# papuSpartan/stable-diffusion-webui-distributed

Hardware: NVIDIA H100
Metric: images/sec SD1.5 512x512 txt2img (higher is better)
Workload: dtype fp16

## Files before the change

### stable-diffusion-webui-distributed_b200/b200sd/csrc/attention_tc.cu

```cuda
#include <cstddef>
#include <cstdlib>

#include "tc_common.cuh"
#include "wgmma.cuh"
#include "b200sd_internal.h"
#include "pdl.cuh"

namespace b200sd {

constexpr int kAttnMathThreads = 256;
constexpr int kAttnThreads = kAttnMathThreads + 128;
constexpr int kQTile = 128;
constexpr int kMaxStages = 3;
constexpr uint32_t kQChunkBytes = kQTile * 128;
__host__ __device__ constexpr int kv_tile(int chunks) { return chunks == 1 ? 128 : 64; }

struct AttnParams {
  int B, heads, Sq, Skv, d, d_pad;
  int d16;
  int chunks;
  int stages;
  float scale_log2;
  void* O;
  long long ldo;
  const int* kv_len;
};

struct __align__(8) AttnShared {
  uint64_t q_full;
  uint64_t kv_full[kMaxStages];
  uint64_t kv_empty[kMaxStages];
};

template <bool kBf16>
__device__ __forceinline__ uint32_t pack_h2(float a, float b) {
  if constexpr (kBf16) {
    __nv_bfloat162 v = __floats2bfloat162_rn(a, b);
    return *reinterpret_cast<uint32_t*>(&v);
  } else {
    __half2 v = __floats2half2_rn(a, b);
    return *reinterpret_cast<uint32_t*>(&v);
  }
}

__device__ __forceinline__ void turn_wait(int wg) {
  asm volatile("bar.sync %0, %1;" ::"r"(2 + wg), "n"(kAttnMathThreads) : "memory");
}
__device__ __forceinline__ void turn_pass(int wg) {
  asm volatile("bar.arrive %0, %1;" ::"r"(3 - wg), "n"(kAttnMathThreads) : "memory");
}

template <int kKv, bool kMask>
__device__ __forceinline__ void softmax_tile(float (&s)[kKv / 2], float (&m_run)[2], float (&l_run)[2],
                                             float (&alpha)[2], float c, int valid, int colq) {
  float mx[2] = {-INFINITY, -INFINITY};
#pragma unroll
  for (int g = 0; g < kKv / 8; ++g)
#pragma unroll
    for (int h = 0; h < 2; ++h)
#pragma unroll
      for (int e = 0; e < 2; ++e) {
        float& v = s[4 * g + 2 * h + e];
        if constexpr (kMask) v = (8 * g + colq + e < valid) ? v : -INFINITY;
        mx[h] = fmaxf(mx[h], v);
      }
  float mc[2];
#pragma unroll
  for (int h = 0; h < 2; ++h) {
    mx[h] = fmaxf(mx[h], __shfl_xor_sync(0xffffffffu, mx[h], 1));
    mx[h] = fmaxf(mx[h], __shfl_xor_sync(0xffffffffu, mx[h], 2));
    const float m_new = fmaxf(m_run[h], mx[h]);
    alpha[h] = fast_exp2((m_run[h] - m_new) * c);
    m_run[h] = m_new;
    mc[h] = m_new * c;
    l_run[h] *= alpha[h];
  }
#pragma unroll
  for (int g = 0; g < kKv / 8; ++g)
#pragma unroll
    for (int h = 0; h < 2; ++h) {
      float& p0 = s[4 * g + 2 * h];
      float& p1 = s[4 * g + 2 * h + 1];
      p0 = fast_exp2(fmaf(p0, c, -mc[h]));
      p1 = fast_exp2(fmaf(p1, c, -mc[h]));
      l_run[h] += p0 + p1;
    }
}

template <int kSteps, int kKv, bool kBf16>
__device__ __forceinline__ void qk_tile(float (&s)[kKv / 2], uint64_t dq, uint64_t dk) {
#pragma unroll
  for (int ks = 0; ks < kSteps; ++ks) {
    const uint32_t off = static_cast<uint32_t>(ks & 3) * 32u;
    Wgmma<kKv, kBf16>::ss(s, dq + ((static_cast<uint32_t>(ks >> 2) * kQChunkBytes + off) >> 4),
                          dk + ((static_cast<uint32_t>(ks >> 2) * (kKv * 128u) + off) >> 4), ks != 0 ? 1u : 0u);
  }
}

template <int kChunks, bool kBf16, bool kVarlen>
__global__ void __launch_bounds__(kAttnThreads, 1)
attention_tc_kernel(const __grid_constant__ CUtensorMap tmQ, const __grid_constant__ CUtensorMap tmK,
                    const __grid_constant__ CUtensorMap tmV, const AttnParams p) {
  constexpr int kKv = kv_tile(kChunks);
  constexpr int kDv = 64 * kChunks;
  constexpr bool kOverlap = kChunks < 3;
  constexpr uint32_t kKvChunkBytes = kKv * 128;
  constexpr uint32_t kKvBytes = kChunks * kKvChunkBytes;
  extern __shared__ uint8_t smem_raw[];
  pdl_trigger();
  uint8_t* smem = reinterpret_cast<uint8_t*>((reinterpret_cast<uintptr_t>(smem_raw) + 1023) & ~uintptr_t(1023));
  uint8_t* sQ = smem;
  uint8_t* sK = sQ + kChunks * kQChunkBytes;
  uint8_t* sV = sK + p.stages * kKvBytes;
  AttnShared* sh = reinterpret_cast<AttnShared*>(sV + p.stages * kKvBytes);

  const int warp = threadIdx.x >> 5;
  const int lane = threadIdx.x & 31;
  const int qt = blockIdx.x;
  const int head = blockIdx.y;
  const int b = blockIdx.z;
  const int col0 = head * p.d_pad;

  if (threadIdx.x == kAttnMathThreads) {
    tma_prefetch_desc(&tmQ);
    tma_prefetch_desc(&tmK);
    tma_prefetch_desc(&tmV);
    mbar_init(&sh->q_full, 1);
    for (int s = 0; s < kMaxStages; ++s) {
      mbar_init(&sh->kv_full[s], 1);
      mbar_init(&sh->kv_empty[s], kAttnMathThreads / 128);
    }
    fence_mbar_init();
  }
  __syncthreads();
  pdl_wait();
  const int skv = kVarlen ? min(max(p.kv_len[b], 1), p.Skv) : p.Skv;
  const int nkv = (skv + kKv - 1) / kKv;

  if (warp >= kAttnMathThreads / 32) {
    producer_warpgroup_regs();
    if (threadIdx.x == kAttnMathThreads) {
      mbar_arrive_expect_tx(&sh->q_full, kChunks * kQChunkBytes);
#pragma unroll
      for (int c = 0; c < kChunks; ++c)
        tma_load_3d(sQ + c * kQChunkBytes, &tmQ, &sh->q_full, col0 + c * 64, qt * kQTile, b);
      for (int t = 0; t < nkv; ++t) {
        const int s = t % p.stages;
        if (t >= p.stages) mbar_wait(&sh->kv_empty[s], static_cast<uint32_t>(t / p.stages - 1) & 1u);
        mbar_arrive_expect_tx(&sh->kv_full[s], 2 * kKvBytes);
#pragma unroll
        for (int c = 0; c < kChunks; ++c) {
          tma_load_3d(sK + s * kKvBytes + c * kKvChunkBytes, &tmK, &sh->kv_full[s], col0 + c * 64, t * kKv, b);
          tma_load_3d(sV + s * kKvBytes + c * kKvChunkBytes, &tmV, &sh->kv_full[s], col0 + c * 64, t * kKv, b);
        }
      }
    }
    return;
  }

  consumer_warpgroup_regs();
  const int wg = warp >> 2;
  const int colq = (lane & 3) * 2;
  const bool signaller = (threadIdx.x & 127) == 0;
  const float c = p.scale_log2;
  const bool ragged = skv % kKv != 0;
  const uint32_t sQ_a = smem_u32(sQ) + static_cast<uint32_t>(wg) * 8192u;
  const uint32_t sK_a = smem_u32(sK), sV_a = smem_u32(sV);
  float o[kDv / 2];
#pragma unroll
  for (int i = 0; i < kDv / 2; ++i) o[i] = 0.f;
  float m_run[2] = {-INFINITY, -INFINITY}, l_run[2] = {0.f, 0.f}, alpha[2];
  float sacc[kKv / 2];
  uint32_t pa[kKv / 16][4];

  auto issue_qk = [&](int t) {
    const uint64_t dq = make_gdesc_sw128(sQ_a, 16, 1024);
    const uint64_t dk = make_gdesc_sw128(sK_a + static_cast<uint32_t>(t % p.stages) * kKvBytes, 16, 1024);
    switch (p.d16 / 16 - 4 * kChunks) {
      case -3: qk_tile<4 * kChunks - 3, kKv, kBf16>(sacc, dq, dk); break;
      case -2: qk_tile<4 * kChunks - 2, kKv, kBf16>(sacc, dq, dk); break;
      case -1: qk_tile<4 * kChunks - 1, kKv, kBf16>(sacc, dq, dk); break;
      default: qk_tile<4 * kChunks, kKv, kBf16>(sacc, dq, dk); break;
    }
    wgmma_commit();
  };
  auto issue_pv = [&](int t) {
    const uint64_t dv = make_gdesc_sw128(sV_a + static_cast<uint32_t>(t % p.stages) * kKvBytes, kKvChunkBytes, 1024);
#pragma unroll
    for (int j = 0; j < kKv / 16; ++j) Wgmma<kDv, kBf16>::rs_tb(o, pa[j], dv + static_cast<uint32_t>(j) * (2048u >> 4), 1u);
    wgmma_commit();
  };
  auto softmax = [&](int t) {
    if (ragged && t == nkv - 1) softmax_tile<kKv, true>(sacc, m_run, l_run, alpha, c, skv - t * kKv, colq);
    else softmax_tile<kKv, false>(sacc, m_run, l_run, alpha, c, 0, colq);
  };
  auto pack_p = [&]() {
#pragma unroll
    for (int g = 0; g < kKv / 8; ++g)
#pragma unroll
      for (int h = 0; h < 2; ++h) pa[g >> 1][(g & 1) * 2 + h] = pack_h2<kBf16>(sacc[4 * g + 2 * h], sacc[4 * g + 2 * h + 1]);
  };

  if (wg == 1) turn_pass(wg);
  mbar_wait(&sh->q_full, 0);
  mbar_wait(&sh->kv_full[0], 0);
  turn_wait(wg);
  wgmma_fence();
  issue_qk(0);
  turn_pass(wg);
  wgmma_wait<0>();
  reg_fence(sacc);
  softmax(0);
  pack_p();

  for (int t = 1; t < nkv; ++t) {
    mbar_wait(&sh->kv_full[t % p.stages], static_cast<uint32_t>(t / p.stages) & 1u);
    turn_wait(wg);
    reg_fence(o);
    wgmma_fence();
    if constexpr (kOverlap) {
      issue_qk(t);
      issue_pv(t - 1);
    } else {
      issue_pv(t - 1);
      wgmma_wait<0>();
      reg_fence(o);
      wgmma_fence();
      issue_qk(t);
    }
    turn_pass(wg);
    wgmma_wait<kOverlap ? 1 : 0>();
    reg_fence(sacc);
    softmax(t);
    wgmma_wait<0>();
    reg_fence(o);
    if (signaller) mbar_arrive(&sh->kv_empty[(t - 1) % p.stages]);
#pragma unroll
    for (int i = 0; i < kDv / 2; ++i) o[i] *= alpha[(i >> 1) & 1];
    pack_p();
  }

  turn_wait(wg);
  reg_fence(o);
  wgmma_fence();
  issue_pv(nkv - 1);
  if (wg == 0) turn_pass(wg);
  wgmma_wait<0>();
  reg_fence(o);
  if (signaller) mbar_arrive(&sh->kv_empty[(nkv - 1) % p.stages]);

#pragma unroll
  for (int h = 0; h < 2; ++h) {
    l_run[h] += __shfl_xor_sync(0xffffffffu, l_run[h], 1);
    l_run[h] += __shfl_xor_sync(0xffffffffu, l_run[h], 2);
  }
  const int r0 = qt * kQTile + wg * 64 + (warp & 3) * 16 + (lane >> 2);
#pragma unroll
  for (int h = 0; h < 2; ++h) {
    const int row = r0 + 8 * h;
    if (row >= p.Sq) continue;
    const float inv = 1.0f / l_run[h];
    uint8_t* orow = static_cast<uint8_t*>(p.O) + ((static_cast<long long>(b) * p.Sq + row) * p.ldo +
                                                  static_cast<long long>(head) * p.d) * 2;
#pragma unroll
    for (int g = 0; g < kDv / 8; ++g) {
      const int col = 8 * g + colq;
      if (col < p.d)
        *reinterpret_cast<uint32_t*>(orow + col * 2) = pack_h2<kBf16>(o[4 * g + 2 * h] * inv, o[4 * g + 2 * h + 1] * inv);
    }
  }
}

typedef void (*AttnKernel)(CUtensorMap, CUtensorMap, CUtensorMap, AttnParams);

template <bool kVarlen>
static AttnKernel attn_kernel_for(int chunks, int is_bf16) {
  switch (chunks * 2 + (is_bf16 ? 1 : 0)) {
    case 2: return attention_tc_kernel<1, false, kVarlen>;
    case 3: return attention_tc_kernel<1, true, kVarlen>;
    case 4: return attention_tc_kernel<2, false, kVarlen>;
    case 5: return attention_tc_kernel<2, true, kVarlen>;
    case 6: return attention_tc_kernel<3, false, kVarlen>;
    case 7: return attention_tc_kernel<3, true, kVarlen>;
    default: return nullptr;
  }
}

static int g_attn_max_smem = 0;
static bool g_attn_dev_ready[64] = {};

int attention_tc(const void* Q, long long ldq, const void* K, long long ldk, const void* V, long long ldv, void* O,
                 long long ldo, int B, int heads, int Sq, int Skv, const int* kv_len, int d, int d_pad, float scale,
                 int v_ones_col, int is_bf16, cudaStream_t stream) {
  if (B <= 0 || heads <= 0 || Sq <= 0) return B200SD_OK;
  if (Skv <= 0 || d <= 0 || d % 8 != 0 || d_pad % 16 != 0 || d_pad < d) return B200SD_ERR_INVALID;
  if (ldq % 8 || ldk % 8 || ldv % 8 || ldo % 8) return B200SD_ERR_INVALID;
  if ((reinterpret_cast<uintptr_t>(Q) | reinterpret_cast<uintptr_t>(K) | reinterpret_cast<uintptr_t>(V) |
       reinterpret_cast<uintptr_t>(O)) & 15)
    return B200SD_ERR_INVALID;
  if (ldq < static_cast<long long>(heads) * d_pad || ldk < static_cast<long long>(heads) * d_pad ||
      ldv < static_cast<long long>(heads) * d_pad || ldo < static_cast<long long>(heads) * d)
    return B200SD_ERR_INVALID;
  if (v_ones_col && d >= d_pad) return B200SD_ERR_INVALID;
  if (kv_len && (reinterpret_cast<uintptr_t>(kv_len) & 3)) return B200SD_ERR_INVALID;
  const int chunks = (((d + 15) & ~15) + 63) / 64;
  if (chunks > 3) return B200SD_ERR_UNSUPPORTED;
  {
    int dev = 0;
    if (cudaGetDevice(&dev) != cudaSuccess) return B200SD_ERR_CUDA;
    if (dev < 0 || dev >= 64) return B200SD_ERR_UNSUPPORTED;
    if (!g_attn_dev_ready[dev]) {
      int smem = 0;
      if (cudaDeviceGetAttribute(&smem, cudaDevAttrMaxSharedMemoryPerBlockOptin, dev) != cudaSuccess)
        return B200SD_ERR_CUDA;
      for (int c = 1; c <= 3; ++c)
        for (int bf = 0; bf < 2; ++bf)
          if (cudaFuncSetAttribute(attn_kernel_for<false>(c, bf), cudaFuncAttributeMaxDynamicSharedMemorySize, smem) !=
                  cudaSuccess ||
              cudaFuncSetAttribute(attn_kernel_for<true>(c, bf), cudaFuncAttributeMaxDynamicSharedMemorySize, smem) !=
                  cudaSuccess)
            return B200SD_ERR_CUDA;
      g_attn_max_smem = smem;
      g_attn_dev_ready[dev] = true;
    }
  }
  AttnParams p{};
  p.B = B; p.heads = heads; p.Sq = Sq; p.Skv = Skv; p.d = d; p.d_pad = d_pad;
  p.d16 = (d + 15) & ~15;
  p.chunks = chunks;
  p.scale_log2 = scale * 1.4426950408889634f;
  p.O = O; p.ldo = ldo;
  p.kv_len = kv_len;
  const int kv = kv_tile(chunks);
  const int nkv = (Skv + kv - 1) / kv;
  const size_t qt = static_cast<size_t>(chunks) * kQChunkBytes;
  const size_t kvt = 2 * static_cast<size_t>(chunks) * kv * 128;
  p.stages = nkv < kMaxStages ? nkv : kMaxStages;
  const size_t smem = 1024 + qt + static_cast<size_t>(p.stages) * kvt + sizeof(AttnShared);
  if (smem > static_cast<size_t>(g_attn_max_smem)) return B200SD_ERR_UNSUPPORTED;
  CUtensorMap tmQ, tmK, tmV;
  const uint32_t es[3] = {1, 1, 1};
  int rc;
  {
    const uint32_t box[3] = {64, kQTile, 1};
    const uint64_t dims[3] = {static_cast<uint64_t>(heads) * d_pad, static_cast<uint64_t>(Sq), static_cast<uint64_t>(B)};
    const uint64_t st[2] = {static_cast<uint64_t>(ldq) * 2, static_cast<uint64_t>(ldq) * 2 * Sq};
    if ((rc = make_tmap_sw128(&tmQ, Q, 3, dims, st, box, es)) != B200SD_OK) return rc;
  }
  const uint32_t kvbox[3] = {64, static_cast<uint32_t>(kv), 1};
  {
    const uint64_t dims[3] = {static_cast<uint64_t>(heads) * d_pad, static_cast<uint64_t>(Skv), static_cast<uint64_t>(B)};
    const uint64_t st[2] = {static_cast<uint64_t>(ldk) * 2, static_cast<uint64_t>(ldk) * 2 * Skv};
    if ((rc = make_tmap_sw128(&tmK, K, 3, dims, st, kvbox, es)) != B200SD_OK) return rc;
  }
  {
    const uint64_t dims[3] = {static_cast<uint64_t>(heads) * d_pad, static_cast<uint64_t>(Skv), static_cast<uint64_t>(B)};
    const uint64_t st[2] = {static_cast<uint64_t>(ldv) * 2, static_cast<uint64_t>(ldv) * 2 * Skv};
    if ((rc = make_tmap_sw128(&tmV, V, 3, dims, st, kvbox, es)) != B200SD_OK) return rc;
  }
  dim3 grid((Sq + kQTile - 1) / kQTile, heads, B);
  launch_pdl(kv_len ? attn_kernel_for<true>(chunks, is_bf16) : attn_kernel_for<false>(chunks, is_bf16), grid, dim3(kAttnThreads), smem, stream, tmQ, tmK, tmV, p);
  return cudaGetLastError() == cudaSuccess ? B200SD_OK : B200SD_ERR_CUDA;
}

}
```

### stable-diffusion-webui-distributed_b200/b200sd/csrc/tc_common.cuh

```cuda
#pragma once
#include <cuda.h>
#include <cuda_bf16.h>
#include <cuda_fp16.h>
#include <cuda_runtime.h>
#include <stdint.h>
#include <stdio.h>
#include "../../../include/b200sd.h"

namespace b200sd {

__device__ __forceinline__ uint32_t smem_u32(const void* p) {
  return static_cast<uint32_t>(__cvta_generic_to_shared(p));
}

__device__ __forceinline__ float fast_exp2(float x) {
  float y;
  asm("ex2.approx.ftz.f32 %0, %1;" : "=f"(y) : "f"(x));
  return y;
}

__device__ __forceinline__ void mbar_init(uint64_t* bar, uint32_t count) {
  asm volatile("mbarrier.init.shared::cta.b64 [%0], %1;" ::"r"(smem_u32(bar)), "r"(count) : "memory");
}
__device__ __forceinline__ void fence_mbar_init() {
  asm volatile("fence.mbarrier_init.release.cluster;" ::: "memory");
}
__device__ __forceinline__ void mbar_arrive_expect_tx(uint64_t* bar, uint32_t bytes) {
  asm volatile("mbarrier.arrive.expect_tx.shared::cta.b64 _, [%0], %1;" ::"r"(smem_u32(bar)), "r"(bytes)
               : "memory");
}
__device__ __forceinline__ void mbar_arrive(uint64_t* bar) {
  asm volatile("mbarrier.arrive.shared::cta.b64 _, [%0];" ::"r"(smem_u32(bar)) : "memory");
}
#ifndef B200SD_WAIT_HINT_NS
#define B200SD_WAIT_HINT_NS 20000
#endif
__device__ __forceinline__ bool mbar_try_wait(uint64_t* bar, uint32_t parity) {
  uint32_t ok;
  asm volatile(
      "{\n\t"
      ".reg .pred P;\n\t"
      "mbarrier.try_wait.parity.shared::cta.b64 P, [%1], %2, %3;\n\t"
      "selp.b32 %0, 1, 0, P;\n\t"
      "}\n"
      : "=r"(ok)
      : "r"(smem_u32(bar)), "r"(parity), "r"(static_cast<uint32_t>(B200SD_WAIT_HINT_NS))
      : "memory");
  return ok != 0;
}
#ifndef B200SD_SPIN_LIMIT
#define B200SD_SPIN_LIMIT (1u << 22)
#endif
__device__ __forceinline__ void mbar_wait(uint64_t* bar, uint32_t parity) {
  uint32_t spins = 0;
  while (!mbar_try_wait(bar, parity)) {
    if (++spins > B200SD_SPIN_LIMIT) __trap();
  }
}

__device__ __forceinline__ void tma_prefetch_desc(const CUtensorMap* m) {
  asm volatile("prefetch.tensormap [%0];" ::"l"(reinterpret_cast<uint64_t>(m)) : "memory");
}
__device__ __forceinline__ void tma_load_2d(void* dst, const CUtensorMap* m, uint64_t* bar, int c0, int c1) {
  asm volatile(
      "cp.async.bulk.tensor.2d.shared::cluster.global.mbarrier::complete_tx::bytes [%0], [%1, {%3, %4}], [%2];"
      ::"r"(smem_u32(dst)), "l"(reinterpret_cast<uint64_t>(m)), "r"(smem_u32(bar)), "r"(c0), "r"(c1)
      : "memory");
}
__device__ __forceinline__ void tma_load_3d(void* dst, const CUtensorMap* m, uint64_t* bar, int c0, int c1, int c2) {
  asm volatile(
      "cp.async.bulk.tensor.3d.shared::cluster.global.mbarrier::complete_tx::bytes [%0], [%1, {%3, %4, %5}], [%2];"
      ::"r"(smem_u32(dst)), "l"(reinterpret_cast<uint64_t>(m)), "r"(smem_u32(bar)), "r"(c0), "r"(c1), "r"(c2)
      : "memory");
}
__device__ __forceinline__ void tma_load_4d(void* dst, const CUtensorMap* m, uint64_t* bar, int c0, int c1, int c2,
                                            int c3) {
  asm volatile(
      "cp.async.bulk.tensor.4d.shared::cluster.global.mbarrier::complete_tx::bytes [%0], [%1, {%3, %4, %5, %6}], "
      "[%2];" ::"r"(smem_u32(dst)),
      "l"(reinterpret_cast<uint64_t>(m)), "r"(smem_u32(bar)), "r"(c0), "r"(c1), "r"(c2), "r"(c3)
      : "memory");
}

__device__ __forceinline__ void fence_proxy_async_smem() { asm volatile("fence.proxy.async.shared::cta;" ::: "memory"); }

__device__ __forceinline__ void wgmma_fence() { asm volatile("wgmma.fence.sync.aligned;" ::: "memory"); }
__device__ __forceinline__ void wgmma_commit() { asm volatile("wgmma.commit_group.sync.aligned;" ::: "memory"); }
template <int N>
__device__ __forceinline__ void wgmma_wait() {
  asm volatile("wgmma.wait_group.sync.aligned %0;" ::"n"(N) : "memory");
}
template <int N>
__device__ __forceinline__ void setmaxnreg_inc() {
  asm volatile("setmaxnreg.inc.sync.aligned.u32 %0;" ::"n"(N) : "memory");
}
template <int N>
__device__ __forceinline__ void setmaxnreg_dec() {
  asm volatile("setmaxnreg.dec.sync.aligned.u32 %0;" ::"n"(N) : "memory");
}
__device__ __forceinline__ void producer_warpgroup_regs() { setmaxnreg_dec<40>(); }
__device__ __forceinline__ void consumer_warpgroup_regs() { setmaxnreg_inc<232>(); }
template <int N>
__device__ __forceinline__ void reg_fence(float (&d)[N]) {
#pragma unroll
  for (int i = 0; i < N; ++i) asm volatile("" : "+f"(d[i])::"memory");
}

__device__ __forceinline__ uint64_t make_gdesc_sw128(uint32_t smem_addr, uint32_t lbo_bytes, uint32_t sbo_bytes) {
  uint64_t d = 0;
  d |= static_cast<uint64_t>((smem_addr & 0x3FFFF) >> 4);
  d |= static_cast<uint64_t>((lbo_bytes >> 4) & 0x3FFF) << 16;
  d |= static_cast<uint64_t>((sbo_bytes >> 4) & 0x3FFF) << 32;
  d |= static_cast<uint64_t>(1) << 62;
  return d;
}

__host__ __device__ __forceinline__ uint32_t sw128_offset(uint32_t row, uint32_t chunk16) {
  return row * 128u + (((chunk16 ^ (row & 7u)) & 7u) << 4);
}

__host__ __device__ __forceinline__ uint32_t sw64_offset(uint32_t row, uint32_t chunk16) {
  return row * 64u + (((chunk16 ^ ((row >> 1) & 3u)) & 3u) << 4);
}

__device__ __forceinline__ void tma_store_2d(const CUtensorMap* m, const void* src, int c0, int c1) {
  asm volatile("cp.async.bulk.tensor.2d.global.shared::cta.bulk_group [%0, {%2, %3}], [%1];" ::"l"(
                   reinterpret_cast<uint64_t>(m)),
               "r"(smem_u32(src)), "r"(c0), "r"(c1)
               : "memory");
}
__device__ __forceinline__ void tma_store_4d(const CUtensorMap* m, const void* src, int c0, int c1, int c2, int c3) {
  asm volatile("cp.async.bulk.tensor.4d.global.shared::cta.bulk_group [%0, {%2, %3, %4, %5}], [%1];" ::"l"(
                   reinterpret_cast<uint64_t>(m)),
               "r"(smem_u32(src)), "r"(c0), "r"(c1), "r"(c2), "r"(c3)
               : "memory");
}
__device__ __forceinline__ void bulk_commit() { asm volatile("cp.async.bulk.commit_group;" ::: "memory"); }
template <int N>
__device__ __forceinline__ void bulk_wait_read() {
  asm volatile("cp.async.bulk.wait_group.read %0;" ::"n"(N) : "memory");
}
template <int N>
__device__ __forceinline__ void bulk_wait() {
  asm volatile("cp.async.bulk.wait_group %0;" ::"n"(N) : "memory");
}


typedef CUresult (*PFN_encodeTiled)(CUtensorMap*, CUtensorMapDataType, cuuint32_t, void*, const cuuint64_t*,
                                    const cuuint64_t*, const cuuint32_t*, const cuuint32_t*, CUtensorMapInterleave,
                                    CUtensorMapSwizzle, CUtensorMapL2promotion, CUtensorMapFloatOOBfill);
PFN_encodeTiled get_encode_tiled();

int make_tmap_sw128(CUtensorMap* out, const void* base, int rank, const uint64_t* dims, const uint64_t* strides_bytes,
                    const uint32_t* box, const uint32_t* elem_strides);
int make_tmap_sw64(CUtensorMap* out, const void* base, int rank, const uint64_t* dims, const uint64_t* strides_bytes,
                   const uint32_t* box, const uint32_t* elem_strides);

}
```

Measured before the change: 11.54.

## Use three math warpgroups with 192-row Q tiles for head-dim-64 attention

For the single-chunk (head dim ≤64) attention path, the kernel now runs three consumer warpgroups, giving a 192-row Q tile, with the ping-pong turn barrier generalised to rotate across N warpgroups. Register budgets are rebalanced and the KV pipeline gets up to 4 stages. Stage/phase tracking replaces per-iteration modulo/divide, the softmax row-max uses split partial maxima for ILP, and the consumer waits drop the spin-limit trap check. The aim is more K/V reuse per load and better latency hiding, at the cost of fewer CTAs, a lower per-thread register cap (160), and possible tail waste when Sq is not a multiple of 192.

Result: faster. 12.11 (median of 6 runs) (+4.9%).

```diff
diff --git a/stable-diffusion-webui-distributed_b200/b200sd/csrc/attention_tc.cu b/stable-diffusion-webui-distributed_b200/b200sd/csrc/attention_tc.cu
--- a/stable-diffusion-webui-distributed_b200/b200sd/csrc/attention_tc.cu
+++ b/stable-diffusion-webui-distributed_b200/b200sd/csrc/attention_tc.cu
@@ -8,12 +8,12 @@
 
 namespace b200sd {
 
-constexpr int kAttnMathThreads = 256;
-constexpr int kAttnThreads = kAttnMathThreads + 128;
-constexpr int kQTile = 128;
-constexpr int kMaxStages = 3;
-constexpr uint32_t kQChunkBytes = kQTile * 128;
+constexpr int kMaxStages = 4;
 __host__ __device__ constexpr int kv_tile(int chunks) { return chunks == 1 ? 128 : 64; }
+__host__ __device__ constexpr int math_warpgroups(int chunks) { return chunks == 1 ? 3 : 2; }
+__host__ __device__ constexpr int q_tile(int chunks) { return 64 * math_warpgroups(chunks); }
+__host__ __device__ constexpr int attn_threads(int chunks) { return 128 * (math_warpgroups(chunks) + 1); }
+__host__ __device__ constexpr int max_stages(int chunks) { return chunks == 1 ? kMaxStages : 3; }
 
 struct AttnParams {
   int B, heads, Sq, Skv, d, d_pad;
@@ -44,16 +44,21 @@
 }
 
 __device__ __forceinline__ void turn_wait(int wg) {
-  asm volatile("bar.sync %0, %1;" ::"r"(2 + wg), "n"(kAttnMathThreads) : "memory");
-}
+  asm volatile("bar.sync %0, %1;" ::"r"(2 + wg), "n"(256) : "memory");
+}
+template <int kMathWg>
 __device__ __forceinline__ void turn_pass(int wg) {
-  asm volatile("bar.arrive %0, %1;" ::"r"(3 - wg), "n"(kAttnMathThreads) : "memory");
+  asm volatile("bar.arrive %0, %1;" ::"r"(2 + (wg + 1) % kMathWg), "n"(256) : "memory");
 }
 
 template <int kKv, bool kMask>
 __device__ __forceinline__ void softmax_tile(float (&s)[kKv / 2], float (&m_run)[2], float (&l_run)[2],
                                              float (&alpha)[2], float c, int valid, int colq) {
-  float mx[2] = {-INFINITY, -INFINITY};
+  float mp[2][4];
+#pragma unroll
+  for (int h = 0; h < 2; ++h)
+#pragma unroll
+    for (int j = 0; j < 4; ++j) mp[h][j] = -INFINITY;
 #pragma unroll
   for (int g = 0; g < kKv / 8; ++g)
 #pragma unroll
@@ -62,11 +67,13 @@
       for (int e = 0; e < 2; ++e) {
         float& v = s[4 * g + 2 * h + e];
         if constexpr (kMask) v = (8 * g + colq + e < valid) ? v : -INFINITY;
-        mx[h] = fmaxf(mx[h], v);
+        float& m = mp[h][2 * (g & 1) + e];
+        m = fmaxf(m, v);
       }
-  float mc[2];
+  float mx[2], mc[2];
 #pragma unroll
   for (int h = 0; h < 2; ++h) {
+    mx[h] = fmaxf(fmaxf(mp[h][0], mp[h][1]), fmaxf(mp[h][2], mp[h][3]));
     mx[h] = fmaxf(mx[h], __shfl_xor_sync(0xffffffffu, mx[h], 1));
     mx[h] = fmaxf(mx[h], __shfl_xor_sync(0xffffffffu, mx[h], 2));
     const float m_new = fmaxf(m_run[h], mx[h]);
@@ -87,7 +94,7 @@
     }
 }
 
-template <int kSteps, int kKv, bool kBf16>
+template <int kSteps, int kKv, uint32_t kQChunkBytes, bool kBf16>
 __device__ __forceinline__ void qk_tile(float (&s)[kKv / 2], uint64_t dq, uint64_t dk) {
 #pragma unroll
   for (int ks = 0; ks < kSteps; ++ks) {
@@ -98,10 +105,14 @@
 }
 
 template <int kChunks, bool kBf16, bool kVarlen>
-__global__ void __launch_bounds__(kAttnThreads, 1)
+__global__ void __launch_bounds__(attn_threads(kChunks), 1)
 attention_tc_kernel(const __grid_constant__ CUtensorMap tmQ, const __grid_constant__ CUtensorMap tmK,
                     const __grid_constant__ CUtensorMap tmV, const AttnParams p) {
   constexpr int kKv = kv_tile(kChunks);
+  constexpr int kMathWg = math_warpgroups(kChunks);
+  constexpr int kMathThreads = 128 * kMathWg;
+  constexpr int kQTile = q_tile(kChunks);
+  constexpr uint32_t kQChunkBytes = kQTile * 128;
   constexpr int kDv = 64 * kChunks;
   constexpr bool kOverlap = kChunks < 3;
   constexpr uint32_t kKvChunkBytes = kKv * 128;
@@ -121,14 +132,14 @@
   const int b = blockIdx.z;
   const int col0 = head * p.d_pad;
 
-  if (threadIdx.x == kAttnMathThreads) {
+  if (threadIdx.x == kMathThreads) {
     tma_prefetch_desc(&tmQ);
     tma_prefetch_desc(&tmK);
     tma_prefetch_desc(&tmV);
     mbar_init(&sh->q_full, 1);
     for (int s = 0; s < kMaxStages; ++s) {
       mbar_init(&sh->kv_full[s], 1);
-      mbar_init(&sh->kv_empty[s], kAttnMathThreads / 128);
+      mbar_init(&sh->kv_empty[s], kMathWg);
     }
     fence_mbar_init();
   }
@@ -137,28 +148,30 @@
   const int skv = kVarlen ? min(max(p.kv_len[b], 1), p.Skv) : p.Skv;
   const int nkv = (skv + kKv - 1) / kKv;
 
-  if (warp >= kAttnMathThreads / 32) {
-    producer_warpgroup_regs();
-    if (threadIdx.x == kAttnMathThreads) {
+  if (warp >= kMathThreads / 32) {
+    setmaxnreg_dec<kMathWg == 3 ? 24 : 40>();
+    if (threadIdx.x == kMathThreads) {
       mbar_arrive_expect_tx(&sh->q_full, kChunks * kQChunkBytes);
 #pragma unroll
       for (int c = 0; c < kChunks; ++c)
         tma_load_3d(sQ + c * kQChunkBytes, &tmQ, &sh->q_full, col0 + c * 64, qt * kQTile, b);
+      int s = 0;
+      uint32_t phase = 0;
       for (int t = 0; t < nkv; ++t) {
-        const int s = t % p.stages;
-        if (t >= p.stages) mbar_wait(&sh->kv_empty[s], static_cast<uint32_t>(t / p.stages - 1) & 1u);
+        if (t >= p.stages) mbar_wait(&sh->kv_empty[s], phase ^ 1u);
         mbar_arrive_expect_tx(&sh->kv_full[s], 2 * kKvBytes);
 #pragma unroll
         for (int c = 0; c < kChunks; ++c) {
           tma_load_3d(sK + s * kKvBytes + c * kKvChunkBytes, &tmK, &sh->kv_full[s], col0 + c * 64, t * kKv, b);
           tma_load_3d(sV + s * kKvBytes + c * kKvChunkBytes, &tmV, &sh->kv_full[s], col0 + c * 64, t * kKv, b);
         }
+        if (++s == p.stages) { s = 0; phase ^= 1u; }
       }
     }
     return;
   }
 
-  consumer_warpgroup_regs();
+  setmaxnreg_inc<kMathWg == 3 ? 160 : 232>();
   const int wg = warp >> 2;
   const int colq = (lane & 3) * 2;
   const bool signaller = (threadIdx.x & 127) == 0;
@@ -173,19 +186,19 @@
   float sacc[kKv / 2];
   uint32_t pa[kKv / 16][4];
 
-  auto issue_qk = [&](int t) {
+  auto issue_qk = [&](int s) {
     const uint64_t dq = make_gdesc_sw128(sQ_a, 16, 1024);
-    const uint64_t dk = make_gdesc_sw128(sK_a + static_cast<uint32_t>(t % p.stages) * kKvBytes, 16, 1024);
+    const uint64_t dk = make_gdesc_sw128(sK_a + static_cast<uint32_t>(s) * kKvBytes, 16, 1024);
     switch (p.d16 / 16 - 4 * kChunks) {
-      case -3: qk_tile<4 * kChunks - 3, kKv, kBf16>(sacc, dq, dk); break;
-      case -2: qk_tile<4 * kChunks - 2, kKv, kBf16>(sacc, dq, dk); break;
-      case -1: qk_tile<4 * kChunks - 1, kKv, kBf16>(sacc, dq, dk); break;
-      default: qk_tile<4 * kChunks, kKv, kBf16>(sacc, dq, dk); break;
+      case -3: qk_tile<4 * kChunks - 3, kKv, kQChunkBytes, kBf16>(sacc, dq, dk); break;
+      case -2: qk_tile<4 * kChunks - 2, kKv, kQChunkBytes, kBf16>(sacc, dq, dk); break;
+      case -1: qk_tile<4 * kChunks - 1, kKv, kQChunkBytes, kBf16>(sacc, dq, dk); break;
+      default: qk_tile<4 * kChunks, kKv, kQChunkBytes, kBf16>(sacc, dq, dk); break;
     }
     wgmma_commit();
   };
-  auto issue_pv = [&](int t) {
-    const uint64_t dv = make_gdesc_sw128(sV_a + static_cast<uint32_t>(t % p.stages) * kKvBytes, kKvChunkBytes, 1024);
+  auto issue_pv = [&](int s) {
+    const uint64_t dv = make_gdesc_sw128(sV_a + static_cast<uint32_t>(s) * kKvBytes, kKvChunkBytes, 1024);
 #pragma unroll
     for (int j = 0; j < kKv / 16; ++j) Wgmma<kDv, kBf16>::rs_tb(o, pa[j], dv + static_cast<uint32_t>(j) * (2048u >> 4), 1u);
     wgmma_commit();
@@ -201,40 +214,44 @@
       for (int h = 0; h < 2; ++h) pa[g >> 1][(g & 1) * 2 + h] = pack_h2<kBf16>(sacc[4 * g + 2 * h], sacc[4 * g + 2 * h + 1]);
   };
 
-  if (wg == 1) turn_pass(wg);
-  mbar_wait(&sh->q_full, 0);
-  mbar_wait(&sh->kv_full[0], 0);
+  if (wg == kMathWg - 1) turn_pass<kMathWg>(wg);
+  int s = 0;
+  uint32_t phase = 0;
+  mbar_wait_unbounded(&sh->q_full, 0);
+  mbar_wait_unbounded(&sh->kv_full[0], 0);
   turn_wait(wg);
   wgmma_fence();
   issue_qk(0);
-  turn_pass(wg);
+  turn_pass<kMathWg>(wg);
   wgmma_wait<0>();
   reg_fence(sacc);
   softmax(0);
   pack_p();
 
   for (int t = 1; t < nkv; ++t) {
-    mbar_wait(&sh->kv_full[t % p.stages], static_cast<uint32_t>(t / p.stages) & 1u);
+    const int s_prev = s;
+    if (++s == p.stages) { s = 0; phase ^= 1u; }
+    mbar_wait_unbounded(&sh->kv_full[s], phase);
     turn_wait(wg);
     reg_fence(o);
     wgmma_fence();
     if constexpr (kOverlap) {
-      issue_qk(t);
-      issue_pv(t - 1);
+      issue_qk(s);
+      issue_pv(s_prev);
     } else {
-      issue_pv(t - 1);
+      issue_pv(s_prev);
       wgmma_wait<0>();
       reg_fence(o);
       wgmma_fence();
-      issue_qk(t);
-    }
-    turn_pass(wg);
+      issue_qk(s);
+    }
+    turn_pass<kMathWg>(wg);
     wgmma_wait<kOverlap ? 1 : 0>();
     reg_fence(sacc);
     softmax(t);
     wgmma_wait<0>();
     reg_fence(o);
-    if (signaller) mbar_arrive(&sh->kv_empty[(t - 1) % p.stages]);
+    if (signaller) mbar_arrive(&sh->kv_empty[s_prev]);
 #pragma unroll
     for (int i = 0; i < kDv / 2; ++i) o[i] *= alpha[(i >> 1) & 1];
     pack_p();
@@ -243,11 +260,11 @@
   turn_wait(wg);
   reg_fence(o);
   wgmma_fence();
-  issue_pv(nkv - 1);
-  if (wg == 0) turn_pass(wg);
+  issue_pv(s);
+  if (wg != kMathWg - 1) turn_pass<kMathWg>(wg);
   wgmma_wait<0>();
   reg_fence(o);
-  if (signaller) mbar_arrive(&sh->kv_empty[(nkv - 1) % p.stages]);
+  if (signaller) mbar_arrive(&sh->kv_empty[s]);
 
 #pragma unroll
   for (int h = 0; h < 2; ++h) {
@@ -333,16 +350,17 @@
   p.kv_len = kv_len;
   const int kv = kv_tile(chunks);
   const int nkv = (Skv + kv - 1) / kv;
-  const size_t qt = static_cast<size_t>(chunks) * kQChunkBytes;
+  const int qtile = q_tile(chunks);
+  const size_t qt = static_cast<size_t>(chunks) * qtile * 128;
   const size_t kvt = 2 * static_cast<size_t>(chunks) * kv * 128;
-  p.stages = nkv < kMaxStages ? nkv : kMaxStages;
+  p.stages = nkv < max_stages(chunks) ? nkv : max_stages(chunks);
   const size_t smem = 1024 + qt + static_cast<size_t>(p.stages) * kvt + sizeof(AttnShared);
   if (smem > static_cast<size_t>(g_attn_max_smem)) return B200SD_ERR_UNSUPPORTED;
   CUtensorMap tmQ, tmK, tmV;
   const uint32_t es[3] = {1, 1, 1};
   int rc;
   {
-    const uint32_t box[3] = {64, kQTile, 1};
+    const uint32_t box[3] = {64, static_cast<uint32_t>(qtile), 1};
     const uint64_t dims[3] = {static_cast<uint64_t>(heads) * d_pad, static_cast<uint64_t>(Sq), static_cast<uint64_t>(B)};
     const uint64_t st[2] = {static_cast<uint64_t>(ldq) * 2, static_cast<uint64_t>(ldq) * 2 * Sq};
     if ((rc = make_tmap_sw128(&tmQ, Q, 3, dims, st, box, es)) != B200SD_OK) return rc;
@@ -358,8 +376,9 @@
     const uint64_t st[2] = {static_cast<uint64_t>(ldv) * 2, static_cast<uint64_t>(ldv) * 2 * Skv};
     if ((rc = make_tmap_sw128(&tmV, V, 3, dims, st, kvbox, es)) != B200SD_OK) return rc;
   }
-  dim3 grid((Sq + kQTile - 1) / kQTile, heads, B);
-  launch_pdl(kv_len ? attn_kernel_for<true>(chunks, is_bf16) : attn_kernel_for<false>(chunks, is_bf16), grid, dim3(kAttnThreads), smem, stream, tmQ, tmK, tmV, p);
+  dim3 grid((Sq + qtile - 1) / qtile, heads, B);
+  launch_pdl(kv_len ? attn_kernel_for<true>(chunks, is_bf16) : attn_kernel_for<false>(chunks, is_bf16), grid,
+             dim3(attn_threads(chunks)), smem, stream, tmQ, tmK, tmV, p);
   return cudaGetLastError() == cudaSuccess ? B200SD_OK : B200SD_ERR_CUDA;
 }
 
diff --git a/stable-diffusion-webui-distributed_b200/b200sd/csrc/tc_common.cuh b/stable-diffusion-webui-distributed_b200/b200sd/csrc/tc_common.cuh
--- a/stable-diffusion-webui-distributed_b200/b200sd/csrc/tc_common.cuh
+++ b/stable-diffusion-webui-distributed_b200/b200sd/csrc/tc_common.cuh
@@ -55,6 +55,10 @@
   uint32_t spins = 0;
   while (!mbar_try_wait(bar, parity)) {
     if (++spins > B200SD_SPIN_LIMIT) __trap();
+  }
+}
+__device__ __forceinline__ void mbar_wait_unbounded(uint64_t* bar, uint32_t parity) {
+  while (!mbar_try_wait(bar, parity)) {
   }
 }
 
```
